# halixness/distributed-3d-diffusion-pytorch

Hardware: AMD Instinct MI355X
Metric: train imgs/sec (whole node), SRN cars 64x64 bs128 (higher is better)
Workload: dtype bf16; 1 GPU; model=XUNet ch128 ch_mult(1,2,2,4) 136.7M params (3DiM, reference xunet.py), global_batch=128, seq_len=4096, image_size=64, per_gpu_batch=128, micro_batch=128, hip_graph=False, parallelism=dp1, dist_backend=none, tuned_gemms=True, backend=hip

## Files before the change

distributed_3d_diffusion_pytorch_amd/ops/_abi.py:

```python
from __future__ import annotations

import ctypes as C

P = C.c_void_p
I = C.c_int
L = C.c_long
F = C.c_float
U64 = C.c_ulonglong
IP = C.POINTER(C.c_int)

SIGNATURES = {
    "d3d_gn_plan": [I, I, I, IP, IP],
    "d3d_gn_cfg": [I, I, I],
    "d3d_gn_cfg_small": [I, I],
    "d3d_gn_stats": [P, I, I, I, I, F, P, P, P, I, P],
    "d3d_gn_apply": [P, P, P, P, P, I, I, I, I, I, P],
    "d3d_gn_film": [P, P, P, P, P, P, I, I, I, I, F, U64, I, P, P],
    "d3d_gn_bwd": [I, P, P, P, P, P, P, I, I, I, I, F, U64, P, P, P, P, P, P, P, P],
    "d3d_ray_dir": [P, P, P, P, I, I, I, I, P],
    "d3d_border_fix": [P, P, I, I, I, I, I, I, I, P, P],
    "d3d_border_sums": [P, P, I, I, I, I, P],
    "d3d_gn_apply2": [I, P, P, P, P, P, P, P, I, I, I, I, F, F, U64, I, P, P, I, I, P, P],
    "d3d_set_words64": [P, I, C.c_longlong, C.c_longlong, C.c_longlong, P],
    "d3d_sgemm_jobs": [P, I, I, P],
    "d3d_gn_ab": [P, P, P, P, P, I, I, I, I, F, I, P],
    "d3d_gn_ab_silu": [P, P, P, I, I, I, P],
    "d3d_gn_img_cfg": [I],
    "d3d_gn_img_ok": [I, I, I],
    "d3d_gn_img_ok_n": [I, I, I, I],
    "d3d_gn_img_wide_cfg": [I, I],
    "d3d_gn_img_fwd": [I, P, P, P, P, P, P, I, I, I, I, F, F, U64, I, P, P, I, P, P],
    "d3d_gn_img_bwd": [I, P, P, P, P, P, P, I, I, I, I, F, U64, P, P, P, I, P, P, P, I, P, F, P, F, P],
    "d3d_gn_bwd2": [I, P, P, P, P, P, P, I, I, I, I, F, U64, P, P, P, P, P, P, P, I, I, P, P, P, I, P, F, P, F, P],
    "d3d_conv_s64_cfg": [I],
    "d3d_conv_hsm_cfg": [I],
    "d3d_gemm_small_k": [I],
    "d3d_gemm_mf": [I],
    "d3d_gemm_w8_waves": [I],
    "d3d_attn_bwd_cfg": [I],
    "d3d_attn_fwd_cfg": [I],
    "d3d_colsum_jobs": [P, I, P],
    "d3d_conv_halo_cfg": [I],
    "d3d_period_sum": [P, P, I, L, P],
    "d3d_silu": [P, P, L, P],
    "d3d_dsilu": [P, P, P, L, P],
    "d3d_avgpool2": [P, P, I, I, I, I, I, P],
    "d3d_upsample2": [P, P, I, I, I, I, I, P],
    "d3d_add_scale": [P, P, P, F, L, P],
    "d3d_set_words": [P, I, F, F, F, F, F, F, F, F, P],
    "d3d_add_scale_gn": [P, P, P, F, L, I, I, I, P, P],
    "d3d_sampler_step": [P, P, P, P, P, I, I, F, F, F, F, F, I, U64, P],
    "d3d_sampler_inputs": [P, P, I, I, P, P, U64, L, P, P, P],
    "d3d_sampler_step2": [P, P, P, I, I, P, P, U64, L, P],
    "d3d_sampler_solve": [P, P, P, P, I, I, P, P, U64, L, P],
    "d3d_randn_hash": [P, L, U64, L, P],
    "d3d_diffusion_fwd2": [P, I, I, U64, P, L, F, F, F, P, P, P, P, P],
    "d3d_diff_loss": [P, P, I, I, I, I, P, P, P],
    "d3d_diff_loss_bwd": [P, P, P, I, I, I, I, P, P],
    "d3d_adam": [P, P, P, P, P, L, F, F, F, F, F, F, F, F, P],
    "d3d_adam_dev": [P, P, P, P, P, L, P, P],
    "d3d_chansum": [P, P, P, P, I, I, I, I, P],
    "d3d_colsum": [P, L, I, P, P, P, I, P],
    "d3d_conv3_gn_ok": [I, I, I, I, I],
    "d3d_conv3_gn": [P, P, P, P, I, I, I, I, I, I, P, I, IP, P, P],
    "d3d_conv3": [P, P, P, P, P, P, I, I, I, I, I, I, I, I, I, I, I, F, I, I, P, I, P, I, IP, P, IP, P],
    "d3d_conv_plan": [I, I, I, I, I, I],
    "d3d_set_wgrad_impl": [I],
    "d3d_conv_wgrad_plan2": [I, I, I, I, I, I, IP, IP],
    "d3d_conv_wgrad_plan3": [I, I, I, I, I, I, I, I, I, IP, IP],
    "d3d_pack_weight": [P, P, I, I, I, I, I, I, P],
    "d3d_set_conv_impl": [I, P],
    "d3d_pack_all": [P, P, I, P],
    "d3d_conv_wgrad_cat": [P, P, P, I, P, P, P, I, I, I, I, I, I, P],
    "d3d_conv_wgrad_seg": [P, P, P, I, I, I, I, I, I, I, I, I, I, I, I, I, P, P, P, P],
    "d3d_wgrad_scatter": [P, I, I, I, I, P, I, I, P, P, P, P],
    "d3d_conv_wgrad3": [P, P, P, P, P, I, I, I, I, I, I, I, I, I, I, I, I, F, P],
    "d3d_ray_posenc": [P, P, P, P, P, P, P, P, I, I, I, P],
    "d3d_cond_prep": [P, P, P, I, C.c_double, C.c_double, P, P, P, P],
    "d3d_attn_fwd": [P, P, P, I, I, I, I, I, F, P],
    "d3d_adam_fused": [P, P, P, P, P, P, P, P, I, P, P, I, I, P],
    "d3d_mlp_ws": [I, I, I],
    "d3d_mlp_pe": [P, I, I, F, P, P],
    "d3d_mlp_mm": [P, P, I, I, I, I, I, I, P, P, P, P, P],
    "d3d_mlp_wgrad": [P, P, I, I, I, I, P, P, I, P],
    "d3d_gemm": [P, P, P, P, I, P, I, I, I, I, I, I, I, F, F, P, I, I, I, P],
    "d3d_gemm_cat": [P, P, P, I, P, P, I, I, I, I, I, F, F, P],
    "d3d_sgemm_strided": [P, P, P, I, I, I, I, L, L, L, L, L, L, L, L, L, F, F, P],
    "d3d_wgrad_tn_plan": [I, I, L, I, I],
    "d3d_wgrad_tn": [P, P, P, P, I, I, L, I, I, I, P],
    "d3d_wgrad_tn_tune": [I],
    "d3d_gemm_nt_ok": [I, I, I, I, I],
    "d3d_gemm_tune": [I, I, I],
    "d3d_gemm_nt": [P, P, P, P, P, I, I, I, I, I, I, I, F, F, P],
    "d3d_gemm_nt_gn": [P, P, P, P, P, I, I, I, I, I, I, I, F, F, P, I, I, P],
    "d3d_attn_bwd": [P, P, P, P, P, P, I, I, I, I, I, F, P],
    "d3d_attn_bwd_slabs": [I, I, I, I],
    "d3d_wgrad_group_cfg": [I, I, I],
    "d3d_wgrad_group_ok": [P],
    "d3d_wgrad_group_stages": [I],
    "d3d_wgrad_group_halo": [I, I, I],
    "d3d_wgrad_group_halo_big": [I, I],
    "d3d_wgrad_group_halo_pk": [I],
    "d3d_wgrad_group_engine": [P],
    "d3d_wgrad_group": [P, I, P, L, P],
    "d3d_wgrad_group_plan": [P, I, IP, IP, C.POINTER(C.c_long)],
    "d3d_image_metrics": [P, P, I, I, I, I, I, C.POINTER(C.c_double), P, P, P],
}


def declare(lib: C.CDLL) -> None:
    for name, args in SIGNATURES.items():
        fn = getattr(lib, name, None)
        if fn is None:
            continue
        fn.argtypes = args
        fn.restype = C.c_long if name in RET_LONG else C.c_int


RET_LONG = {"d3d_mlp_ws", "d3d_wgrad_group"}
```

distributed_3d_diffusion_pytorch_amd/ops/csrc/conv.hip:

```cpp
#include "common.h"
#include <stdlib.h>

#include <algorithm>

D3D_API int d3d_colsum(const float* in, long R, int Cc, float* part, float* out, float* out_odd, int accumulate,
                       hipStream_t st);

typedef __attribute__((ext_vector_type(4))) short s16x4;
typedef __attribute__((ext_vector_type(8))) short s16x8;
typedef __attribute__((address_space(3))) s16x4 lds_s16x4;

namespace {

template <int TAPS, bool TRANS>
__global__ void __launch_bounds__(256, 2)
conv_glds_k(const bf16* __restrict__ I, const bf16* __restrict__ Wp, const float* __restrict__ bias,
            const float* __restrict__ row_bias, const bf16* __restrict__ res, bf16* __restrict__ O,
            const bf16* __restrict__ zero16, int Nimg, int IH, int IW, int IC, int ICp, int OH, int OW, int OC,
            int ldo, int stride, float scale, int res_nmod, float* __restrict__ part, int korder) {
  constexpr int BM = 128, BN = 128, BKk = 64;
  constexpr int WM = 64, WN = 64, TM = 4, TN = 4;
  constexpr int STAGE = (BM + BN) * BKk;
  __shared__ __attribute__((aligned(16))) bf16 smem[2 * STAGE];
  typedef __attribute__((address_space(3))) void lds_void;
// ... 558 lines not shown
  constexpr int NH = WN / 64;
  float gs[TM][NH], gq[TM][NH];
#pragma unroll
  for (int i = 0; i < TM; ++i)
#pragma unroll
    for (int h = 0; h < NH; ++h) gs[i][h] = gq[i][h] = 0.f;
  float cb[TM][4];
#pragma unroll
  for (int i = 0; i < TM; ++i) {
    const int co = m0 + wm * WM + i * 16 + fq * 4;
#pragma unroll
    for (int e = 0; e < 4; ++e) cb[i][e] = (bias && co + e < OC) ? bias[co + e] : 0.f;
  }
#pragma unroll
  for (int j = 0; j < TN; ++j) {
    const long pix = n0 + wn * WN + j * 16 + fr;
    if (pix >= Mpix) continue;
    const int img = (int)(pix / OHW);
    const long rpix = res_nmod > 0 ? (long)(img % res_nmod) * OHW + (pix - (long)img * OHW) : pix;
#pragma unroll
    for (int i = 0; i < TM; ++i) {
      const int co = m0 + wm * WM + i * 16 + fq * 4;
      if (co >= OC) continue;
      float v[4];
#pragma unroll
      for (int e = 0; e < 4; ++e) {
        const int cc = co + e < OC ? co + e : OC - 1;
        float t = acc[i][j][e] + cb[i][e];
        if (row_bias) t += row_bias[(long)img * OC + cc];
        v[e] = t;
      }
      bf16* dst = O + pix * ldo + co;
      if (co + 3 < OC && vec_out) {
        if constexpr (RES) {
          if (res) {
#pragma unroll
            for (int e = 0; e < 4; ++e) v[e] += (float)rres[i][j][e];
          }
        }
        bf16x4 o4;
#pragma unroll
        for (int e = 0; e < 4; ++e) {
          o4[e] = (bf16)(v[e] * scale);
          const float y = (float)o4[e];
          gs[i][j / 4] += y;
          gq[i][j / 4] += y * y;
        }
        *reinterpret_cast<bf16x4*>(dst) = o4;
        if (O2) silu_store4(O2, dst - O, o4);
      } else {
        for (int e = 0; e < 4 && co + e < OC; ++e) {
          float t = v[e];
          if (res) t += (float)res[rpix * ldo + co + e];
          dst[e] = (bf16)(t * scale);
          if (O2) O2[(dst - O) + e] = (bf16)siluf_((float)dst[e]);
          const float y = (float)dst[e];
          gs[i][j / 4] += y;
          gq[i][j / 4] += y * y;
        }
      }
    }
  }
  if (gnp) gn_part_store<TM, NH>(gs, gq, lane, m0 + wm * WM, n0 + wn * WN, OC, gn_groups, OHW, Mpix, gnp);
}

constexpr int HALO_CH = 32;

template <int OWT, int BNT = 512>
struct HaloGeom {
  static constexpr int TR = BNT / OWT;
  static constexpr int HW2 = (OWT + 2 + 7) / 8 * 8;
  static constexpr int HP = (TR + 2) * HW2;
  static constexpr int HPW = (HP + 127) / 128;
  static constexpr int HBUF = HPW * 8 * 16 * HALO_CH;
  static constexpr int ABUF = 128 * HALO_CH;
};

__device__ __forceinline__ void halo_issue_a(bf16* sA, const bf16* Wp, int w_bytes, int aoff, int soff, int wave) {
  typedef __attribute__((address_space(3))) void lds_void;
  const __amdgpu_buffer_rsrc_t rW = __builtin_amdgcn_make_buffer_rsrc((void*)Wp, (short)0, w_bytes, 0x00020000);
  __builtin_amdgcn_raw_ptr_buffer_load_lds(rW, (lds_void*)(sA + wave * 16 * HALO_CH), 16, aoff, soff, 0, 0);
}

template <int HPW>
__device__ __forceinline__ void halo_issue_b(bf16* sH, const bf16* I, int in_bytes, const unsigned* hoff, int cbyte,
                                             int wave) {
  typedef __attribute__((address_space(3))) void lds_void;
  const __amdgpu_buffer_rsrc_t rI = __builtin_amdgcn_make_buffer_rsrc((void*)I, (short)0, in_bytes, 0x00020000);
#pragma unroll
  for (int k = 0; k < HPW; ++k)
    __builtin_amdgcn_raw_ptr_buffer_load_lds(rI, (lds_void*)(sH + (wave + 8 * k) * 16 * HALO_CH), 16,
                                             hoff[k] + (unsigned)cbyte, 0, 0, 0);
}

template <int OWT, bool TRANS, int BNT = 512, bool RES = true, bool P2 = false, bool GNA = false>
__global__ void __launch_bounds__(512, 1)
conv_halo_k(const bf16* __restrict__ I, const bf16* __restrict__ Wp, const float* __restrict__ bias,
            const float* __restrict__ row_bias, const bf16* __restrict__ res, bf16* __restrict__ O, int in_bytes,
            int w_bytes, int Nimg, int OH, int IC, int ICp, int OC, float scale, int res_nmod,
            float* __restrict__ gnp, int gn_groups, bf16* __restrict__ O2, const float* __restrict__ gab) {
  static_assert(!GNA || (!P2 && !TRANS), "GroupNorm staging: forward, single-tap schedule");
  __shared__ __attribute__((aligned(16))) float sG[GNA ? 2 * 512 : 4];
  typedef HaloGeom<OWT, BNT> Gm;
  constexpr int BM = 128, BN = BNT, WM = 64, WN = BN / 4, TM = 4, TN = WN / 16;
  __shared__ __attribute__((aligned(16))) bf16 smem[2 * Gm::HBUF + (P2 ? 8 : 4) * Gm::ABUF];
  bf16* const sH = smem;
  bf16* const sAr = smem + 2 * Gm::HBUF;

  const int tid = threadIdx.x, lane = tid & 63;
  const int wave = __builtin_amdgcn_readfirstlane(tid >> 6);
  const int wm = wave >> 2, wn = wave & 3;
  const int OW = OWT, IH = OH, IW = OW;
  const int tiles = Nimg * (OH / Gm::TR);
  int bid = blockIdx.x;
  {
    int q = tiles / 8, r = tiles % 8, xcd = bid % 8;
    bid = (xcd < r ? xcd * (q + 1) : r * (q + 1) + (xcd - r) * q) + bid / 8;
  }
  const int img = bid / (OH / Gm::TR);
  const int r0 = (bid - img * (OH / Gm::TR)) * Gm::TR;
  const long n0 = ((long)img * OH + r0) * OW;
  const long Mpix = (long)Nimg * OH * OW;
  const int m0 = blockIdx.y * BM;
  const int Kp = 9 * ICp;

  const int arow = wave * 16 + (lane >> 2);
  const int aoff = ((m0 + arow) * Kp + (((lane & 3) ^ ((arow >> 1) & 2)) << 3)) * 2;
  unsigned hoff[Gm::HPW];
#pragma unroll
  for (int k = 0; k < Gm::HPW; ++k) {
    const int fi = (wave + 8 * k) * 16 + (lane >> 2);
    const int hr = fi / Gm::HW2, hc = fi - hr * Gm::HW2;
    const int ih = r0 - 1 + hr, iw = hc - 1;
    const bool ok = fi < Gm::HP && ih >= 0 && ih < IH && iw >= 0 && iw < IW;
    const int q = (lane & 3) ^ ((fi >> 1) & 2);
    const unsigned o = (unsigned)((((img * IH + (ok ? ih : 0)) * IW + (ok ? iw : 0)) * IC + q * 8) * 2);
    hoff[k] = ok ? o : 0x80000000u;
  }
  const int gnq = (lane & 3) ^ ((lane >> 3) & 2);
  auto gn_apply = [&](bf16* hb, int c) {
    if constexpr (GNA) {
      int lo = lane * 8 + wave * 16 * HALO_CH, to = (c * HALO_CH + gnq * 8) * 2;
      asm volatile("" : "+v"(lo), "+v"(to));
      const f32x4* t = reinterpret_cast<const f32x4*>(sG + to);
#pragma unroll
      for (int k = 0; k < Gm::HPW; ++k) {
        const bool ok = hoff[k] != 0x80000000u;
        bf16x2* q = reinterpret_cast<bf16x2*>(hb + lo + 8 * k * 16 * HALO_CH);
#pragma unroll
        for (int h = 0; h < 4; ++h) {
          const f32x4 a = t[h];
          const bf16x2 v = q[h];
          bf16x2 o;
          o[0] = (bf16)siluf_(__builtin_fmaf((float)v[0], a[0], a[1]));
          o[1] = (bf16)siluf_(__builtin_fmaf((float)v[1], a[2], a[3]));
          q[h] = ok ? o : v;
          __builtin_amdgcn_sched_barrier(0);
        }
      }
      asm volatile("s_waitcnt lgkmcnt(0)" ::: "memory");
    }
  };

  const int NCH = IC / HALO_CH, S = 9 * NCH;
  auto a_soff = [&](int s) {
    const int ss = s < S ? s : S - 1;
    const int c = ss / 9, t = ss - c * 9;
    return (t * ICp + c * HALO_CH) * 2;
  };

  f32x4 acc[TM][TN];
#pragma unroll
  for (int i = 0; i < TM; ++i)
#pragma unroll
    for (int j = 0; j < TN; ++j) acc[i][j] = f32x4{0.f, 0.f, 0.f, 0.f};

  const int fr = lane & 15, fq = lane >> 4;
  int hp0[TN];
#pragma unroll
  for (int j = 0; j < TN; ++j) {
    const int p = wn * WN + j * 16 + fr;
    hp0[j] = (p / OWT) * Gm::HW2 + (p % OWT);
  }
  const int OHW = OH * OW;
  if (RES && res) {
#pragma unroll
    for (int j = 0; j < TN; ++j) {
      const long pix = n0 + wn * WN + j * 16 + fr;
      const long rpix = res_nmod > 0 ? (long)(img % res_nmod) * OHW + (pix - (long)img * OHW) : pix;
#pragma unroll
      for (int i = 0; i < TM; ++i) {
        const int co = m0 + wm * WM + i * 16 + fq * 4;
        const bf16x4 r4 = co < OC ? *reinterpret_cast<const bf16x4*>(res + rpix * OC + co) : bf16x4{};
#pragma unroll
        for (int e = 0; e < 4; ++e) acc[i][j][e] = (float)r4[e];
      }
    }
  }

  if constexpr (P2) {
  halo_issue_b<Gm::HPW>(sH, I, in_bytes, hoff, 0, wave);
#pragma unroll
  for (int k = 0; k < 4; ++k) halo_issue_a(sAr + k * Gm::ABUF, Wp, w_bytes, aoff, a_soff(k), wave);
  int bo[3][TN], ao[TM];
#pragma unroll
  for (int kw = 0; kw < 3; ++kw)
#pragma unroll
    for (int j = 0; j < TN; ++j) {
      const int hp = hp0[j] + kw;
      bo[kw][j] = hp * HALO_CH + ((fq ^ ((hp >> 1) & 2)) << 3);
    }
#pragma unroll
  for (int i = 0; i < TM; ++i) {
    const int row = wm * WM + i * 16 + fr;
    ao[i] = row * HALO_CH + ((fq ^ ((row >> 1) & 2)) << 3);
  }
  auto step = [&](int s, int t, const bf16* hb) {
    const bf16* a = sAr + (s & 7) * Gm::ABUF;
    const int kh = TRANS ? 2 - t / 3 : t / 3, kw = TRANS ? 2 - t % 3 : t % 3;
    bf16x8 af[TM], bfr[TN];
#pragma unroll
    for (int j = 0; j < TN; ++j) bfr[j] = *reinterpret_cast<const bf16x8*>(hb + kh * Gm::HW2 * HALO_CH + bo[kw][j]);
#pragma unroll
    for (int i = 0; i < TM; ++i) af[i] = *reinterpret_cast<const bf16x8*>(a + ao[i]);
#pragma unroll
    for (int i = 0; i < TM; ++i)
#pragma unroll
      for (int j = 0; j < TN; ++j)
        acc[i][j] = __builtin_amdgcn_mfma_f32_16x16x32_bf16(af[i], bfr[j], acc[i][j], 0, 0, 0);
  };
  for (int c2 = 0; c2 < NCH; c2 += 2) {
    const int S0 = c2 * 9;
#pragma unroll
    for (int pp = 0; pp < 9; ++pp) {
      if (pp == 1 || pp == 2 || pp == 6 || pp == 7) {
        asm volatile("s_waitcnt vmcnt(%0)" ::"n"(2 + Gm::HPW) : "memory");
      } else {
        asm volatile("s_waitcnt vmcnt(2)" ::: "memory");
      }
      __builtin_amdgcn_s_barrier();
      const int s0 = S0 + 2 * pp;
      halo_issue_a(sAr + ((s0 + 4) & 7) * Gm::ABUF, Wp, w_bytes, aoff, a_soff(s0 + 4), wave);
      halo_issue_a(sAr + ((s0 + 5) & 7) * Gm::ABUF, Wp, w_bytes, aoff, a_soff(s0 + 5), wave);
      if (pp == 0 || pp == 5) {
        const int cn0 = c2 + (pp == 0 ? 1 : 2), cn = cn0 < NCH ? cn0 : NCH - 1;
        halo_issue_b<Gm::HPW>(sH + (cn0 & 1) * Gm::HBUF, I, in_bytes, hoff, cn * HALO_CH * 2, wave);
      }
      __builtin_amdgcn_s_setprio(1);
      const int sr0 = 2 * pp, sr1 = 2 * pp + 1;
      step(S0 + sr0, sr0 % 9, sH + (sr0 / 9) * Gm::HBUF);
      step(S0 + sr1, sr1 % 9, sH + (sr1 / 9) * Gm::HBUF);
      __builtin_amdgcn_s_setprio(0);
    }
  }
  } else {
  float gt[GNA ? 2 : 1];
  if constexpr (GNA) {
#pragma unroll
    for (int i = 0; i < 2; ++i) {
      const int j = tid + 512 * i;
      gt[i] = j < 2 * IC ? gab[(long)img * IC * 2 + j] : 0.f;
    }
  }
  halo_issue_b<Gm::HPW>(sH, I, in_bytes, hoff, 0, wave);
  halo_issue_a(sAr, Wp, w_bytes, aoff, a_soff(0), wave);
  halo_issue_a(sAr + Gm::ABUF, Wp, w_bytes, aoff, a_soff(1), wave);
  halo_issue_a(sAr + 2 * Gm::ABUF, Wp, w_bytes, aoff, a_soff(2), wave);
  if constexpr (GNA) {
#pragma unroll
    for (int i = 0; i < 2; ++i) sG[tid + 512 * i] = gt[i];
  }
  asm volatile("s_waitcnt vmcnt(0)" ::: "memory");
  if constexpr (GNA) {
    asm volatile("s_waitcnt lgkmcnt(0)" ::: "memory");
    __builtin_amdgcn_s_barrier();
    gn_apply(sH, 0);
  }
  int bo[3][TN], ao[TM];
#pragma unroll
  for (int kw = 0; kw < 3; ++kw)
#pragma unroll
    for (int j = 0; j < TN; ++j) {
      const int hp = hp0[j] + kw;
      bo[kw][j] = hp * HALO_CH + ((fq ^ ((hp >> 1) & 2)) << 3);
    }
#pragma unroll
  for (int i = 0; i < TM; ++i) {
    const int row = wm * WM + i * 16 + fr;
    ao[i] = row * HALO_CH + ((fq ^ ((row >> 1) & 2)) << 3);
  }
  for (int c = 0; c < NCH; ++c) {
    const bf16* hb = sH + (c & 1) * Gm::HBUF;
#pragma unroll
    for (int t = 0; t < 9; ++t) {
      const int s = c * 9 + t;
      if (t >= 1 && t <= 3) {
        asm volatile("s_waitcnt vmcnt(%0)" ::"n"(2 + Gm::HPW) : "memory");
      } else {
        asm volatile("s_waitcnt vmcnt(2)" ::: "memory");
      }
      __builtin_amdgcn_s_barrier();
      halo_issue_a(sAr + ((s + 3) & 3) * Gm::ABUF, Wp, w_bytes, aoff, a_soff(s + 3), wave);
      if (t == 0) {
        const int cn = c + 1 < NCH ? c + 1 : NCH - 1;
        halo_issue_b<Gm::HPW>(sH + ((c + 1) & 1) * Gm::HBUF, I, in_bytes, hoff, cn * HALO_CH * 2, wave);
      }
      if (t == 4) gn_apply(sH + ((c + 1) & 1) * Gm::HBUF, c + 1 < NCH ? c + 1 : NCH - 1);
      const bf16* a = sAr + (s & 3) * Gm::ABUF;
      __builtin_amdgcn_s_setprio(1);
      bf16x8 af[TM], bfr[TN];
      const int kh = TRANS ? 2 - t / 3 : t / 3, kw = TRANS ? 2 - t % 3 : t % 3;
#pragma unroll
      for (int j = 0; j < TN; ++j) bfr[j] = *reinterpret_cast<const bf16x8*>(hb + kh * Gm::HW2 * HALO_CH + bo[kw][j]);
#pragma unroll
      for (int i = 0; i < TM; ++i) af[i] = *reinterpret_cast<const bf16x8*>(a + ao[i]);
#pragma unroll
      for (int i = 0; i < TM; ++i)
#pragma unroll
        for (int j = 0; j < TN; ++j)
          acc[i][j] = __builtin_amdgcn_mfma_f32_16x16x32_bf16(af[i], bfr[j], acc[i][j], 0, 0, 0);
      __builtin_amdgcn_s_setprio(0);
    }
  }
  }
  asm volatile("s_waitcnt vmcnt(0)" ::: "memory");

  constexpr int NH = WN / 64;
  float gs[TM][NH], gq[TM][NH];
#pragma unroll
  for (int i = 0; i < TM; ++i)
#pragma unroll
    for (int h = 0; h < NH; ++h) gs[i][h] = gq[i][h] = 0.f;
  float cb[TM][4];
#pragma unroll
  for (int i = 0; i < TM; ++i) {
    const int co = m0 + wm * WM + i * 16 + fq * 4;
#pragma unroll
    for (int e = 0; e < 4; ++e) {
      float t = 0.f;
      if (co + e < OC) {
        if (bias) t += bias[co + e];
        if (row_bias) t += row_bias[(long)img * OC + co + e];
      }
      cb[i][e] = t;
    }
  }
#ifdef D3D_HALO_EPI_DIRECT
  constexpr bool LEPI = false;
#else
  constexpr bool LEPI = true;
#endif
  static_assert(2 * Gm::HBUF + (P2 ? 8 : 4) * Gm::ABUF >= BN * 128, "output tile must fit the LDS");
  const bool lepi = LEPI && (OC % 8) == 0;
  bf16* const sT = smem;
  if (lepi) {
    asm volatile("s_waitcnt lgkmcnt(0)" ::: "memory");
    __builtin_amdgcn_s_barrier();
  }
#pragma unroll
  for (int j = 0; j < TN; ++j) {
    const long pix = n0 + wn * WN + j * 16 + fr;
    const int pl = wn * WN + j * 16 + fr;
#pragma unroll
    for (int i = 0; i < TM; ++i) {
      const int co = m0 + wm * WM + i * 16 + fq * 4;
      if (co >= OC) continue;
      float v[4];
#pragma unroll
      for (int e = 0; e < 4; ++e) v[e] = acc[i][j][e] + cb[i][e];
      bf16x4 o4;
#pragma unroll
      for (int e = 0; e < 4; ++e) {
        o4[e] = (bf16)(v[e] * scale);
        const float y = (float)o4[e];
        gs[i][j / 4] += y;
        gq[i][j / 4] += y * y;
      }
      if (lepi) {
        const int cl = wm * WM + i * 16 + fq * 4;
        *reinterpret_cast<bf16x4*>(sT + pl * 128 + (((cl >> 3) ^ (pl & 15)) << 3) + (cl & 4)) = o4;
      } else {
        *reinterpret_cast<bf16x4*>(O + pix * OC + co) = o4;
        if (O2) silu_store4(O2, pix * OC + co, o4);
      }
    }
  }
  if (gnp) gn_part_store<TM, NH>(gs, gq, lane, m0 + wm * WM, n0 + wn * WN, OC, gn_groups, OHW, Mpix, gnp);
  if (lepi) {
    asm volatile("s_waitcnt lgkmcnt(0)" ::: "memory");
    __builtin_amdgcn_s_barrier();
#pragma unroll 4
    for (int idx = tid; idx < BN * 16; idx += 512) {
      const int pl = idx >> 4, c = idx & 15;
      const int co = m0 + c * 8;
      if (co >= OC) continue;
      const bf16x8 v = *reinterpret_cast<const bf16x8*>(sT + pl * 128 + ((c ^ (pl & 15)) << 3));
      const long off = (n0 + pl) * OC + co;
      *reinterpret_cast<bf16x8*>(O + off) = v;
      if (O2) {
        bf16x8 s8;
#pragma unroll
        for (int e = 0; e < 8; ++e) s8[e] = (bf16)siluf_((float)v[e]);
        *reinterpret_cast<bf16x8*>(O2 + off) = s8;
      }
    }
  }
}

__global__ void conv_splitk_epi_k(const float* __restrict__ part, int nsplit, long Mpix, int OC, int OHW,
                                  const float* __restrict__ bias, const float* __restrict__ row_bias,
                                  const bf16* __restrict__ res, int res_nmod, bf16* __restrict__ O, int ldo,
                                  float scale, bf16* __restrict__ O2) {
  const long nv = Mpix * (OC / 4);
  const long slab = Mpix * OC;
  for (long v = blockIdx.x * (long)blockDim.x + threadIdx.x; v < nv; v += (long)gridDim.x * blockDim.x) {
    long pix = v / (OC / 4);
    int co = (int)(v % (OC / 4)) * 4;
    f32x4 a = *reinterpret_cast<const f32x4*>(part + pix * OC + co);
    for (int sp = 1; sp < nsplit; ++sp) a += *reinterpret_cast<const f32x4*>(part + sp * slab + pix * OC + co);
    int img = (int)(pix / OHW);
#pragma unroll
    for (int e = 0; e < 4; ++e) {
      float t = a[e] + (bias ? bias[co + e] : 0.f);
      if (row_bias) t += row_bias[(long)img * OC + co + e];
      a[e] = t;
    }
    if (res) {
      const long rpix = res_nmod > 0 ? (long)(img % res_nmod) * OHW + (pix - (long)img * OHW) : pix;
      bf16x4 r4 = *reinterpret_cast<const bf16x4*>(res + rpix * ldo + co);
#pragma unroll
      for (int e = 0; e < 4; ++e) a[e] += (float)r4[e];
    }
    bf16x4 o4;
#pragma unroll
    for (int e = 0; e < 4; ++e) o4[e] = (bf16)(a[e] * scale);
// ... 1004 lines not shown
__global__ void __launch_bounds__(256) pack_all_k(const PackDesc* __restrict__ descs,
                                                  const int* __restrict__ blk_desc) {
  __shared__ float tile[32 * 16 * 9];
  const PackDesc d = descs[blk_desc[blockIdx.x]];
  const int local = blockIdx.x - d.blk0, tid = threadIdx.x;
  const int ics = d.ICs ? d.ICs : d.IC;
  const int T = d.taps;
  if (d.mode == 2) {
    const int t0 = local * 2048 + tid * 8;
    if (t0 >= d.OC) return;
    bf16x8 o;
#pragma unroll
    for (int e = 0; e < 8; ++e) o[e] = (bf16)(t0 + e < d.OC ? d.src[t0 + e] : 0.f);
    if (t0 + 7 < d.OC && ((reinterpret_cast<uintptr_t>(d.dst + t0) & 15) == 0))
      *reinterpret_cast<bf16x8*>(d.dst + t0) = o;
    else
      for (int e = 0; e < 8 && t0 + e < d.OC; ++e) d.dst[t0 + e] = o[e];
    return;
  }
  if (d.mode == 0) {
    const int ncg = (d.ICp + 255) / 256;
    const int co = local / ncg, ci0 = (local % ncg) * 256;
    const int nci = min(256, d.ICp - ci0);
    for (int k = tid; k < 256 * T; k += 256) {
      const int ci = ci0 + k / T;
      tile[k] = (co < d.OC && ci < d.IC) ? d.src[((long)co * ics + ci) * T + k % T] : 0.f;
    }
    __syncthreads();
    for (int k = tid; k < T * (nci / 8); k += 256) {
      const int tap = k / (nci / 8), c8 = (k % (nci / 8)) * 8;
      bf16x8 o;
#pragma unroll
      for (int e = 0; e < 8; ++e) o[e] = (bf16)tile[(c8 + e) * T + tap];
      *reinterpret_cast<bf16x8*>(d.dst + ((long)co * T + tap) * d.ICp + ci0 + c8) = o;
    }
    return;
  }
  const int nct = (d.OCp + 31) / 32;
  const int co0 = (local % nct) * 32, ci0 = (local / nct) * 16;
  for (int k = tid; k < 32 * 16 * T; k += 256) {
    const int r = k / (16 * T), q = k % (16 * T);
    const int co = co0 + r, ci = ci0 + q / T;
    tile[k] = (co < d.OC && ci < d.IC) ? d.src[((long)co * ics + ci) * T + q % T] : 0.f;
  }
  __syncthreads();
  for (int k = tid; k < 16 * T * 4; k += 256) {
    const int c8 = (k & 3) * 8, rt = k >> 2;
    const int ci = rt / T, tap = rt % T;
    if (ci0 + ci >= d.ICp || co0 + c8 >= d.OCp) continue;
    bf16x8 o;
#pragma unroll
    for (int e = 0; e < 8; ++e) o[e] = (bf16)tile[(c8 + e) * 16 * T + ci * T + tap];
    *reinterpret_cast<bf16x8*>(d.dst + ((long)(ci0 + ci) * T + tap) * (d.ldd ? d.ldd : d.OCp) + co0 + c8) = o;
  }
}

}

D3D_API int d3d_pack_all(const void* descs, const int* blk_desc, int total_blocks, hipStream_t st) {
  if (total_blocks <= 0) return 0;
  hipLaunchKernelGGL(pack_all_k, dim3(total_blocks), dim3(256), 0, st, (const PackDesc*)descs, blk_desc);
  return (int)hipGetLastError();
}

static int g_s64 = 1;
extern "C" int d3d_conv_s64_try(const void* I, const void* Wp, const float* bias, const float* row_bias,
                                const void* res, void* O, int N, int IH, int IW, int IC, int ICp, int OH, int OW,
                                int OC, int ldo, int stride, int trans, float scale, int res_nmod, int taps,
                                float* gnp, int gn_groups, int* gn_done, hipStream_t st, void* O2);
extern "C" int d3d_conv_hsm_try(const void* I, const void* Wp, const float* bias, const float* row_bias,
                                const void* res, void* O, int N, int IH, int IW, int IC, int ICp, int OH, int OW,
                                int OC, int ldo, int stride, int trans, float scale, int res_nmod, int taps,
                                const float* gnp, const void* O2, hipStream_t st);
static const long g_s64_maxb = 160;
static bool s64_wanted(long Mpix, int OC, int ICp, int taps) {
  const long blocks128 = ((Mpix + 127) / 128) * ((OC + 127) / 128);
  const long blocks64 = ((Mpix + 63) / 64) * (OC / 64);
  return g_s64 && OC % 64 == 0 && (taps * ICp) % 64 == 0 && blocks128 <= g_s64_maxb && blocks64 >= 128;
}
static int g_halo_w32 = 1;
static int g_halo_w16 = 1;
static int g_halo_w32s = 1;
static int g_halo_p2 = 1;
D3D_API int d3d_conv_halo_cfg(int cfg) {
  g_halo_w32 = (cfg >> 2) & 1;
  g_halo_w16 = (cfg >> 3) & 1;
  g_halo_w32s = (cfg >> 4) & 1;
  g_halo_p2 = (cfg >> 5) & 1;
  return 0;
}

enum ConvImpl {
  CONV_BUFL = 3,
  CONV_W8 = 4,
  CONV_W8W = 6,
  CONV_W8N = 7,
  CONV_HALO = 8,
};
enum WgradImpl {
  WGRAD_REG = 0,
  WGRAD_BUFL = 5,
  WGRAD_W8 = 6,
};
static int g_conv_impl = CONV_HALO;
static int g_wgrad_impl = WGRAD_W8;
static const bf16* g_zero16 = nullptr;
static const int kConvKorder = 1;

D3D_API int d3d_set_wgrad_impl(int impl) {
  if (impl != WGRAD_REG && impl != WGRAD_BUFL && impl != WGRAD_W8) return (int)hipErrorInvalidValue;
  g_wgrad_impl = impl;
  return 0;
}

D3D_API int d3d_set_conv_impl(int impl, const void* zero16) {
  if (impl != CONV_BUFL && impl != CONV_W8 && impl != CONV_W8W && impl != CONV_W8N && impl != CONV_HALO)
    return (int)hipErrorInvalidValue;
  g_conv_impl = impl;
  if (zero16) g_zero16 = (const bf16*)zero16;
  return 0;
}

D3D_API int d3d_conv_plan(int N, int OH, int OW, int OC, int ICp, int taps) {
  constexpr int BM = 128, BN = 128;
  long Mpix = (long)N * OH * OW;
  long blocks = ((Mpix + BN - 1) / BN) * ((OC + BM - 1) / BM);
  int nk = taps * ICp / 64;
  static const int target = 512;
  if (blocks >= 384 || (OC & 3)) return 1;
  if (s64_wanted(Mpix, OC, ICp, taps)) return 1;
  long want = target / blocks;
  long maxs = nk / 6;
  if (want > maxs) want = maxs;
  if (want > 16) want = 16;
  return want < 2 ? 1 : (int)want;
}

D3D_API int d3d_conv3(const void* I, const void* Wp, const float* bias, const float* row_bias, const void* res,
                      void* O, int N, int IH, int IW, int IC, int ICp, int OH, int OW, int OC, int ldo, int stride,
                      int trans, float scale, int res_nmod, int taps, float* ws, int nsplit, float* gnp,
                      int gn_groups, int* gn_done, void* O2, int* silu_done, hipStream_t st) {
  long Mpix = (long)N * OH * OW;
  if (gn_done) *gn_done = 0;
  if (silu_done) *silu_done = 0;
  if (!silu_done) O2 = nullptr;
  {
    const long img_in = (long)IH * IW * IC * 2, img_out = (long)OH * OW * ldo * 2;
    const long lim = (1L << 31) - (1L << 20);
    if (N > 1 && ((long)N * img_in >= lim || (long)N * img_out >= lim)) {
      long per = lim / std::max(img_in, img_out);
      const int q = res_nmod > 0 ? res_nmod : 1;
      per = per / q * q;
      if (per >= 1) {
        const int parts_per_img = (OH * OW) % 64 == 0 ? OH * OW / 64 : 0;
        int all_gn = 1, all_silu = 1;
        for (int n0 = 0; n0 < N; n0 += (int)per) {
          const int nc = (int)std::min<long>(per, N - n0);
          int d = 0, ds = 0;
          const int rc = d3d_conv3((const char*)I + n0 * img_in, Wp, bias,
                                   row_bias ? row_bias + (long)n0 * OC : nullptr,
                                   res ? (res_nmod > 0 ? res : (const char*)res + n0 * img_out) : nullptr,
                                   (char*)O + n0 * img_out, nc, IH, IW, IC, ICp, OH, OW, OC, ldo, stride, trans, scale,
                                   res_nmod, taps, ws, nsplit,
                                   gnp ? gnp + (long)n0 * gn_groups * parts_per_img * 2 : nullptr, gn_groups,
                                   gn_done ? &d : nullptr, O2 ? (char*)O2 + n0 * img_out : nullptr,
                                   O2 ? &ds : nullptr, st);
          if (rc) return rc;
          all_gn &= d;
          all_silu &= ds;
        }
        if (gn_done) *gn_done = gnp ? all_gn : 0;
        if (silu_done) *silu_done = O2 ? all_silu : 0;
        return 0;
      }
    }
  }
  if (gnp) {
    const int Cg = gn_groups > 0 && OC % gn_groups == 0 ? OC / gn_groups : 0;
    const bool ok = (Cg == 4 || Cg == 8 || Cg == 16 || Cg == 32) && (OH * OW) % 64 == 0 && Mpix % 64 == 0 &&
                    ldo == OC;
    if (!ok) gnp = nullptr;
  }
  constexpr int BM = 128, BN = 128;
  if (nsplit < 1 || !ws) nsplit = 1;
  if (nsplit == 1 && s64_wanted(Mpix, OC, ICp, taps)) {
    const int rh = d3d_conv_hsm_try(I, Wp, bias, row_bias, res, O, N, IH, IW, IC, ICp, OH, OW, OC, ldo, stride, trans,
                                    scale, res_nmod, taps, gnp, O2, st);
    if (rh != 0) return rh < 0 ? -rh : 0;
    const int r = d3d_conv_s64_try(I, Wp, bias, row_bias, res, O, N, IH, IW, IC, ICp, OH, OW, OC, ldo, stride, trans,
                                   scale, res_nmod, taps, gnp, gn_groups, gn_done, st, O2);
    if (r > 0 && silu_done) *silu_done = O2 ? 1 : 0;
    if (r != 0) return r < 0 ? -r : 0;
  }
  dim3 grid((unsigned)((Mpix + BN - 1) / BN), (unsigned)((OC + BM - 1) / BM), (unsigned)nsplit);
  const long in_bytes = (long)N * IH * IW * IC * 2, w_bytes = (long)((OC + 127) / 128 * 128) * taps * ICp * 2;
  if (g_conv_impl == CONV_HALO && taps == 9 && stride == 1 && IW == OW && IH == OH && ldo == OC && IC % HALO_CH == 0 &&
      OC % 128 == 0 && (OW == 16 || OW == 32 || OW == 64 || OW == 128) && in_bytes < (1L << 31) &&
      w_bytes < (1L << 31)) {
    auto nblk = [&](int bn) { return OH % (bn / OW) ? 0L : (long)N * (OH / (bn / OW)) * (OC / 128); };
    if ((OW != 32 || g_halo_w32) && nblk(512) >= 256) {
      dim3 gh((unsigned)(N * (OH / (512 / OW))), (unsigned)(OC / 128), 1);
#define HALO3(OWv, TR, RS, P2v)                                                                                   \
  hipLaunchKernelGGL((conv_halo_k<OWv, TR, 512, RS, (P2v && OWv != 128)>), gh, dim3(512), 0, st, (const bf16*)I,  \
                     (const bf16*)Wp, bias, row_bias, (const bf16*)res, (bf16*)O, (int)in_bytes, (int)w_bytes, N, OH, \
                     IC, ICp, OC, scale, res_nmod, gnp, gn_groups, (bf16*)O2, (const float*)nullptr)
#define HALO(OWv, TR, RS)                                                                                          \
  do {                                                                                                            \
    if (g_halo_p2 && OWv != 128 && (IC / HALO_CH) % 2 == 0) HALO3(OWv, TR, RS, true);                             \
    else HALO3(OWv, TR, RS, false);                                                                               \
  } while (0)
      if (OW == 64) {
        if (trans) { if (res) HALO(64, true, true); else HALO(64, true, false); }
        else if (res) HALO(64, false, true); else HALO(64, false, false);
      } else if (OW == 32) {
        if (trans) { if (res) HALO(32, true, true); else HALO(32, true, false); }
        else if (res) HALO(32, false, true); else HALO(32, false, false);
      } else {
        if (trans) { if (res) HALO(128, true, true); else HALO(128, true, false); }
        else if (res) HALO(128, false, true); else HALO(128, false, false);
      }
#undef HALO
#undef HALO3
      if (gn_done && gnp) *gn_done = 1;
      if (silu_done && O2) *silu_done = 1;
      return (int)hipGetLastError();
    }
    if (((OW == 16 && g_halo_w16) || (OW == 32 && g_halo_w32s)) && nblk(256) >= 256) {
      dim3 gh((unsigned)(N * (OH / (256 / OW))), (unsigned)(OC / 128), 1);
#define HALOS(OWv, TR, RS)                                                                                         \
  hipLaunchKernelGGL((conv_halo_k<OWv, TR, 256, RS>), gh, dim3(512), 0, st, (const bf16*)I,                        \
                     (const bf16*)Wp, bias, row_bias, (const bf16*)res, (bf16*)O, (int)in_bytes, (int)w_bytes, N, OH, \
                     IC, ICp, OC, scale, res_nmod, gnp, gn_groups, (bf16*)O2, (const float*)nullptr)
      if (OW == 16) {
        if (trans) { if (res) HALOS(16, true, true); else HALOS(16, true, false); }
        else if (res) HALOS(16, false, true); else HALOS(16, false, false);
      } else {
        if (trans) { if (res) HALOS(32, true, true); else HALOS(32, true, false); }
        else if (res) HALOS(32, false, true); else HALOS(32, false, false);
      }
#undef HALOS
      if (gn_done && gnp) *gn_done = 1;
      if (silu_done && O2) *silu_done = 1;
      return (int)hipGetLastError();
    }
  }
  if (g_conv_impl >= CONV_W8 && (!trans || stride == 1) && in_bytes < (1L << 31) && w_bytes < (1L << 31) && OC >= 64) {
    const int bm = (OC % 256 == 0 || OC > 384) ? 256 : 128;
    const bool wide = bm == 128 && g_conv_impl >= CONV_W8W;
    int bn = wide ? 512 : 256;
    long ptiles = (Mpix + bn - 1) / bn;
    long blocks = ptiles * ((OC + bm - 1) / bm);
    if (g_conv_impl == CONV_W8N && bm == 256 && blocks < 256 && ((Mpix + 127) / 128) * ((OC + 255) / 256) >= 256) {
      bn = 128;
      ptiles = (Mpix + bn - 1) / bn;
      blocks = ptiles * ((OC + bm - 1) / bm);
    }
    if ((bm == 256 || wide) && blocks >= 256) {
      dim3 g8((unsigned)ptiles, (unsigned)((OC + bm - 1) / bm), 1);
#define W8R(TP, TR, BMv, BNv, RS)                                                                                \
  hipLaunchKernelGGL((conv_w8_k<TP, TR, BMv, BNv, RS>), g8, dim3(512), 0, st, (const bf16*)I, (const bf16*)Wp, bias, \
                     row_bias, (const bf16*)res, (bf16*)O, (int)in_bytes, (int)w_bytes, N, IH, IW, IC, ICp, OH, OW, \
                     OC, ldo, stride, scale, res_nmod, kConvKorder, gnp, gn_groups, (bf16*)O2)
#define W8(TP, TR, BMv, BNv)                                                                                     \
  do {                                                                                                          \
    if (res) W8R(TP, TR, BMv, BNv, true); else W8R(TP, TR, BMv, BNv, false);                                     \
  } while (0)
      if (bn == 128) {
        if (taps == 9) {
          if (trans) W8(9, true, 256, 128); else W8(9, false, 256, 128);
        } else {
          if (trans) W8(1, true, 256, 128); else W8(1, false, 256, 128);
        }
      } else if (bm == 256) {
        if (taps == 9) {
          if (trans) W8(9, true, 256, 256); else W8(9, false, 256, 256);
        } else {
          if (trans) W8(1, true, 256, 256); else W8(1, false, 256, 256);
        }
      } else {
        if (taps == 9) {
          if (trans) W8(9, true, 128, 512); else W8(9, false, 128, 512);
        } else {
          if (trans) W8(1, true, 128, 512); else W8(1, false, 128, 512);
        }
      }
#undef W8
#undef W8R
      if (gn_done && gnp) *gn_done = 1;
      if (silu_done && O2) *silu_done = 1;
      return (int)hipGetLastError();
    }
  }
  if ((!trans || stride == 1) && in_bytes < (1L << 31) && w_bytes < (1L << 31)) {
    float* part = nsplit > 1 ? ws : nullptr;
#define BUFL(TP, TR)                                                                                             \
  hipLaunchKernelGGL((conv_bufl_k<TP, TR>), grid, dim3(256), 0, st, (const bf16*)I, (const bf16*)Wp, bias,        \
                     row_bias, (const bf16*)res, (bf16*)O, (int)in_bytes, (int)w_bytes, N, IH, IW, IC, ICp, OH, OW, \
                     OC, ldo, stride, scale, res_nmod, part, kConvKorder, part ? nullptr : gnp, gn_groups,         \
                     part ? nullptr : (bf16*)O2)
    if (taps == 9) {
      if (trans) BUFL(9, true); else BUFL(9, false);
    } else {
      if (trans) BUFL(1, true); else BUFL(1, false);
    }
#undef BUFL
    if (part && gnp && OC % 64 == 0) {
      hipLaunchKernelGGL(conv_splitk_epi_gn_k, dim3((unsigned)(Mpix / 64), (unsigned)(OC / 64)), dim3(256), 0, st,
                         part, nsplit, Mpix, OC, OH * OW, bias, row_bias, (const bf16*)res, res_nmod, (bf16*)O,
                         scale, gnp, gn_groups, (bf16*)O2);
      if (gn_done) *gn_done = 1;
    } else if (part) {
      long nv = Mpix * (OC / 4);
      long g = (nv + 255) / 256;
      if (g > 4096) g = 4096;
      hipLaunchKernelGGL(conv_splitk_epi_k, dim3((unsigned)g), dim3(256), 0, st, part, nsplit, Mpix, OC, OH * OW,
                         bias, row_bias, (const bf16*)res, res_nmod, (bf16*)O, ldo, scale, (bf16*)O2);
    } else if (gn_done && gnp) {
      *gn_done = 1;
    }
    if (silu_done && O2) *silu_done = 1;
    return (int)hipGetLastError();
  }
  if (!g_zero16) return (int)hipErrorInvalidValue;
// ... 314 lines not shown
```

Baseline: 1126 examples/s.

## Add paired 256-pixel halo conv tile with 3-slot weight ring for two workgroups/CU

Adds a variant of the halo 3x3 conv kernel that uses a 256-pixel tile, a 3-slot weight ring instead of 4 slots, and exactly sized halo buffers with a dump slot for overflow loads. This keeps LDS per workgroup under 80 KiB so two 512-thread workgroups can share a CU. A heuristic picks it for OW 32/64 layers with small channel counts and enough blocks. It also adds force/telemetry knobs and an occupancy query. The shallower ring and smaller tile cut prefetch depth and per-block reuse, and the heuristic may send layers to the wrong variant.

After: 1115 examples/s. 1.0% lower.

```diff
diff --git a/distributed_3d_diffusion_pytorch_amd/ops/_abi.py b/distributed_3d_diffusion_pytorch_amd/ops/_abi.py
--- a/distributed_3d_diffusion_pytorch_amd/ops/_abi.py
+++ b/distributed_3d_diffusion_pytorch_amd/ops/_abi.py
@@ -41,6 +41,8 @@
     "d3d_attn_fwd_cfg": [I],
     "d3d_colsum_jobs": [P, I, P],
     "d3d_conv_halo_cfg": [I],
+    "d3d_conv_halo_pair_occupancy": [I, I, I],
+    "d3d_conv_halo_last_tile": [],
     "d3d_period_sum": [P, P, I, L, P],
     "d3d_silu": [P, P, L, P],
     "d3d_dsilu": [P, P, P, L, P],
diff --git a/distributed_3d_diffusion_pytorch_amd/ops/csrc/conv.hip b/distributed_3d_diffusion_pytorch_amd/ops/csrc/conv.hip
--- a/distributed_3d_diffusion_pytorch_amd/ops/csrc/conv.hip
+++ b/distributed_3d_diffusion_pytorch_amd/ops/csrc/conv.hip
@@ -664,30 +664,41 @@
   __builtin_amdgcn_raw_ptr_buffer_load_lds(rW, (lds_void*)(sA + wave * 16 * HALO_CH), 16, aoff, soff, 0, 0);
 }
 
-template <int HPW>
+template <int HPW, int NPC = 8 * HPW>
 __device__ __forceinline__ void halo_issue_b(bf16* sH, const bf16* I, int in_bytes, const unsigned* hoff, int cbyte,
-                                             int wave) {
+                                             int wave, bf16* dump = nullptr) {
   typedef __attribute__((address_space(3))) void lds_void;
   const __amdgpu_buffer_rsrc_t rI = __builtin_amdgcn_make_buffer_rsrc((void*)I, (short)0, in_bytes, 0x00020000);
 #pragma unroll
-  for (int k = 0; k < HPW; ++k)
-    __builtin_amdgcn_raw_ptr_buffer_load_lds(rI, (lds_void*)(sH + (wave + 8 * k) * 16 * HALO_CH), 16,
-                                             hoff[k] + (unsigned)cbyte, 0, 0, 0);
-}
-
-template <int OWT, bool TRANS, int BNT = 512, bool RES = true, bool P2 = false, bool GNA = false>
-__global__ void __launch_bounds__(512, 1)
+  for (int k = 0; k < HPW; ++k) {
+    bf16* dst = sH + (wave + 8 * k) * 16 * HALO_CH;
+    if (8 * k + 7 >= NPC) dst = wave + 8 * k < NPC ? dst : dump;
+    __builtin_amdgcn_raw_ptr_buffer_load_lds(rI, (lds_void*)dst, 16, hoff[k] + (unsigned)cbyte, 0, 0, 0);
+  }
+}
+
+template <int OWT, bool TRANS, int BNT = 512, bool RES = true, bool P2 = false, bool GNA = false,
+          int NW = (P2 ? 8 : 4)>
+__global__ void __launch_bounds__(512, NW == 3 ? 2 : 1)
 conv_halo_k(const bf16* __restrict__ I, const bf16* __restrict__ Wp, const float* __restrict__ bias,
             const float* __restrict__ row_bias, const bf16* __restrict__ res, bf16* __restrict__ O, int in_bytes,
             int w_bytes, int Nimg, int OH, int IC, int ICp, int OC, float scale, int res_nmod,
             float* __restrict__ gnp, int gn_groups, bf16* __restrict__ O2, const float* __restrict__ gab) {
   static_assert(!GNA || (!P2 && !TRANS), "GroupNorm staging: forward, single-tap schedule");
+  constexpr bool PAIR = NW == 3;
+  static_assert(NW == (P2 ? 8 : 4) || (PAIR && BNT == 256 && !P2 && !GNA), "3-slot ring: the paired 256-pixel tile");
   __shared__ __attribute__((aligned(16))) float sG[GNA ? 2 * 512 : 4];
   typedef HaloGeom<OWT, BNT> Gm;
   constexpr int BM = 128, BN = BNT, WM = 64, WN = BN / 4, TM = 4, TN = WN / 16;
-  __shared__ __attribute__((aligned(16))) bf16 smem[2 * Gm::HBUF + (P2 ? 8 : 4) * Gm::ABUF];
+  constexpr int NPC = PAIR ? Gm::HP / 16 : 8 * Gm::HPW;
+  static_assert(!PAIR || (Gm::HP % 16 == 0 && Gm::HW2 % 8 == 0), "whole pieces; kh shifts keep the swizzle");
+  constexpr int HB = NPC * 16 * HALO_CH;
+  constexpr int SMEM = 2 * HB + NW * Gm::ABUF + (PAIR ? 16 * HALO_CH : 0);
+  static_assert(!PAIR || SMEM * 2 <= 81920, "paired tile: two workgroups per CU need <= 80 KiB of LDS each");
+  __shared__ __attribute__((aligned(16))) bf16 smem[SMEM];
   bf16* const sH = smem;
-  bf16* const sAr = smem + 2 * Gm::HBUF;
+  bf16* const sAr = smem + 2 * HB;
+  bf16* const sDump = smem + 2 * HB + NW * Gm::ABUF;
 
   const int tid = threadIdx.x, lane = tid & 63;
   const int wave = __builtin_amdgcn_readfirstlane(tid >> 6);
@@ -844,10 +855,10 @@
       gt[i] = j < 2 * IC ? gab[(long)img * IC * 2 + j] : 0.f;
     }
   }
-  halo_issue_b<Gm::HPW>(sH, I, in_bytes, hoff, 0, wave);
+  halo_issue_b<Gm::HPW, NPC>(sH, I, in_bytes, hoff, 0, wave, sDump);
   halo_issue_a(sAr, Wp, w_bytes, aoff, a_soff(0), wave);
   halo_issue_a(sAr + Gm::ABUF, Wp, w_bytes, aoff, a_soff(1), wave);
-  halo_issue_a(sAr + 2 * Gm::ABUF, Wp, w_bytes, aoff, a_soff(2), wave);
+  if constexpr (NW > 3) halo_issue_a(sAr + 2 * Gm::ABUF, Wp, w_bytes, aoff, a_soff(2), wave);
   if constexpr (GNA) {
 #pragma unroll
     for (int i = 0; i < 2; ++i) sG[tid + 512 * i] = gt[i];
@@ -872,23 +883,23 @@
     ao[i] = row * HALO_CH + ((fq ^ ((row >> 1) & 2)) << 3);
   }
   for (int c = 0; c < NCH; ++c) {
-    const bf16* hb = sH + (c & 1) * Gm::HBUF;
+    const bf16* hb = sH + (c & 1) * HB;
 #pragma unroll
     for (int t = 0; t < 9; ++t) {
       const int s = c * 9 + t;
-      if (t >= 1 && t <= 3) {
-        asm volatile("s_waitcnt vmcnt(%0)" ::"n"(2 + Gm::HPW) : "memory");
+      if (t >= 1 && t <= NW - 1) {
+        asm volatile("s_waitcnt vmcnt(%0)" ::"n"(NW - 2 + Gm::HPW) : "memory");
       } else {
-        asm volatile("s_waitcnt vmcnt(2)" ::: "memory");
+        asm volatile("s_waitcnt vmcnt(%0)" ::"n"(NW - 2) : "memory");
       }
       __builtin_amdgcn_s_barrier();
-      halo_issue_a(sAr + ((s + 3) & 3) * Gm::ABUF, Wp, w_bytes, aoff, a_soff(s + 3), wave);
+      halo_issue_a(sAr + (PAIR ? (t + 2) % 3 : (s + 3) & 3) * Gm::ABUF, Wp, w_bytes, aoff, a_soff(s + (NW - 1)), wave);
       if (t == 0) {
         const int cn = c + 1 < NCH ? c + 1 : NCH - 1;
-        halo_issue_b<Gm::HPW>(sH + ((c + 1) & 1) * Gm::HBUF, I, in_bytes, hoff, cn * HALO_CH * 2, wave);
-      }
-      if (t == 4) gn_apply(sH + ((c + 1) & 1) * Gm::HBUF, c + 1 < NCH ? c + 1 : NCH - 1);
-      const bf16* a = sAr + (s & 3) * Gm::ABUF;
+        halo_issue_b<Gm::HPW, NPC>(sH + ((c + 1) & 1) * HB, I, in_bytes, hoff, cn * HALO_CH * 2, wave, sDump);
+      }
+      if (t == 4) gn_apply(sH + ((c + 1) & 1) * HB, c + 1 < NCH ? c + 1 : NCH - 1);
+      const bf16* a = sAr + (PAIR ? t % 3 : s & 3) * Gm::ABUF;
       __builtin_amdgcn_s_setprio(1);
       bf16x8 af[TM], bfr[TN];
       const int kh = TRANS ? 2 - t / 3 : t / 3, kw = TRANS ? 2 - t % 3 : t % 3;
@@ -932,7 +943,7 @@
 #else
   constexpr bool LEPI = true;
 #endif
-  static_assert(2 * Gm::HBUF + (P2 ? 8 : 4) * Gm::ABUF >= BN * 128, "output tile must fit the LDS");
+  static_assert(SMEM >= BN * 128, "output tile must fit the LDS");
   const bool lepi = LEPI && (OC % 8) == 0;
   bf16* const sT = smem;
   if (lepi) {
@@ -2103,12 +2114,39 @@
 static int g_halo_w16 = 1;
 static int g_halo_w32s = 1;
 static int g_halo_p2 = 1;
+static int g_halo_pair = 1;
+static int g_halo_force = 0;
+static int g_halo_last = 0;
+D3D_API int d3d_conv_halo_last_tile() { return g_halo_last; }
 D3D_API int d3d_conv_halo_cfg(int cfg) {
+  const int prev = (g_halo_w32 << 2) | (g_halo_w16 << 3) | (g_halo_w32s << 4) | (g_halo_p2 << 5) |
+                   (g_halo_pair << 6) | (g_halo_force << 7);
   g_halo_w32 = (cfg >> 2) & 1;
   g_halo_w16 = (cfg >> 3) & 1;
   g_halo_w32s = (cfg >> 4) & 1;
   g_halo_p2 = (cfg >> 5) & 1;
-  return 0;
+  g_halo_pair = (cfg >> 6) & 1;
+  g_halo_force = (cfg >> 7) & 3;
+  return prev;
+}
+static bool halo_pair_wins(int OW, int IC, int OC, int trans, bool res) {
+  if (OW == 64) return IC <= 128 || (IC <= 256 && !trans && !res);
+  return IC <= 256 && !(trans && res && OC > 256);
+}
+
+template <int OWT, bool TRANS, bool RES>
+static int halo_pair_occ_of() {
+  int n = 0;
+  const hipError_t e = hipOccupancyMaxActiveBlocksPerMultiprocessor(
+      &n, conv_halo_k<OWT, TRANS, 256, RES, false, false, 3>, 512, 0);
+  return e == hipSuccess ? n : -(int)e;
+}
+D3D_API int d3d_conv_halo_pair_occupancy(int OW, int trans, int res) {
+  if (OW != 32 && OW != 64) return -(int)hipErrorInvalidValue;
+#define OCC(OWv) (trans ? (res ? halo_pair_occ_of<OWv, true, true>() : halo_pair_occ_of<OWv, true, false>())     \
+                        : (res ? halo_pair_occ_of<OWv, false, true>() : halo_pair_occ_of<OWv, false, false>()))
+  return OW == 64 ? OCC(64) : OCC(32);
+#undef OCC
 }
 
 enum ConvImpl {
@@ -2162,6 +2200,7 @@
                       int trans, float scale, int res_nmod, int taps, float* ws, int nsplit, float* gnp,
                       int gn_groups, int* gn_done, void* O2, int* silu_done, hipStream_t st) {
   long Mpix = (long)N * OH * OW;
+  g_halo_last = 0;
   if (gn_done) *gn_done = 0;
   if (silu_done) *silu_done = 0;
   if (!silu_done) O2 = nullptr;
@@ -2204,7 +2243,7 @@
   }
   constexpr int BM = 128, BN = 128;
   if (nsplit < 1 || !ws) nsplit = 1;
-  if (nsplit == 1 && s64_wanted(Mpix, OC, ICp, taps)) {
+  if (nsplit == 1 && !g_halo_force && s64_wanted(Mpix, OC, ICp, taps)) {
     const int rh = d3d_conv_hsm_try(I, Wp, bias, row_bias, res, O, N, IH, IW, IC, ICp, OH, OW, OC, ldo, stride, trans,
                                     scale, res_nmod, taps, gnp, O2, st);
     if (rh != 0) return rh < 0 ? -rh : 0;
@@ -2219,7 +2258,28 @@
       OC % 128 == 0 && (OW == 16 || OW == 32 || OW == 64 || OW == 128) && in_bytes < (1L << 31) &&
       w_bytes < (1L << 31)) {
     auto nblk = [&](int bn) { return OH % (bn / OW) ? 0L : (long)N * (OH / (bn / OW)) * (OC / 128); };
-    if ((OW != 32 || g_halo_w32) && nblk(512) >= 256) {
+    if ((OW == 32 || OW == 64) && nblk(256) > 0 && (OW != 32 || g_halo_w32 || g_halo_force == 1) &&
+        (g_halo_force == 1 ||
+         (!g_halo_force && g_halo_pair && nblk(256) >= 512 && halo_pair_wins(OW, IC, OC, trans, res != nullptr)))) {
+      dim3 gh((unsigned)(N * (OH / (256 / OW))), (unsigned)(OC / 128), 1);
+#define HALOP(OWv, TR, RS)                                                                                         \
+  hipLaunchKernelGGL((conv_halo_k<OWv, TR, 256, RS, false, false, 3>), gh, dim3(512), 0, st, (const bf16*)I,       \
+                     (const bf16*)Wp, bias, row_bias, (const bf16*)res, (bf16*)O, (int)in_bytes, (int)w_bytes, N, OH, \
+                     IC, ICp, OC, scale, res_nmod, gnp, gn_groups, (bf16*)O2, (const float*)nullptr)
+      if (OW == 64) {
+        if (trans) { if (res) HALOP(64, true, true); else HALOP(64, true, false); }
+        else if (res) HALOP(64, false, true); else HALOP(64, false, false);
+      } else {
+        if (trans) { if (res) HALOP(32, true, true); else HALOP(32, true, false); }
+        else if (res) HALOP(32, false, true); else HALOP(32, false, false);
+      }
+#undef HALOP
+      g_halo_last = 1;
+      if (gn_done && gnp) *gn_done = 1;
+      if (silu_done && O2) *silu_done = 1;
+      return (int)hipGetLastError();
+    }
+    if (((OW != 32 || g_halo_w32) && nblk(512) >= 256) || (g_halo_force == 2 && OW != 16 && nblk(512) > 0)) {
       dim3 gh((unsigned)(N * (OH / (512 / OW))), (unsigned)(OC / 128), 1);
 #define HALO3(OWv, TR, RS, P2v)                                                                                   \
   hipLaunchKernelGGL((conv_halo_k<OWv, TR, 512, RS, (P2v && OWv != 128)>), gh, dim3(512), 0, st, (const bf16*)I,  \
@@ -2242,6 +2302,7 @@
       }
 #undef HALO
 #undef HALO3
+      g_halo_last = 2;
       if (gn_done && gnp) *gn_done = 1;
       if (silu_done && O2) *silu_done = 1;
       return (int)hipGetLastError();
@@ -2260,6 +2321,7 @@
         else if (res) HALOS(32, false, true); else HALOS(32, false, false);
       }
 #undef HALOS
+      g_halo_last = 3;
       if (gn_done && gnp) *gn_done = 1;
       if (silu_done && O2) *silu_done = 1;
       return (int)hipGetLastError();
```
